# remydubois/illico

Measured on NVIDIA B200. Metric: gene_x_group_tests_per_s, higher is better.
Workload: dtype f32 keys / int64 ranks / f64 epilogue

## Files before the change

### illico_b200/csrc/fused.cu

```cuda
#include "common.cuh"
#include "epilogue.cuh"
#include "tma.cuh"

#include <stdlib.h>

namespace illico {

int launch_stage_dense_list(const float* X, long long ld, int gene_lb, const int* list, const int* n_list_dev, const int* mode_dev,
                            int want_mode, const illico_plan_t* plan, float* ir_vals, uint32_t* ir_cnt, cudaStream_t stream);
int launch_stage_dense_tma_if(const float* X, long long ld, int gene_lb, int b, const illico_plan_t* plan, float* ir_vals,
                              uint32_t* ir_cnt, int seg_lo, int seg_hi, cudaStream_t stream, int segs_per_cta_req,
                              const int* mode_dev, int want_mode);
int launch_stage_csr_if(const float*, const int32_t*, const long long*, int, int, const illico_plan_t*, float*, uint32_t*, void*, size_t,
                        const int*, int, cudaStream_t);
int launch_stage_csr_list(const float*, const int32_t*, const long long*, int, int, const int*, const int*, int, int,
                          const illico_plan_t*, float*, uint32_t*, cudaStream_t);
int launch_ovo_mapped(const float*, const uint32_t*, int, const int*, const int*, int, const illico_plan_t*, const illico_flags_t*, double*,
                      long long, void*, size_t, const illico_debug_t*, cudaStream_t);
int launch_ovr_mapped(const float*, const uint32_t*, int, const int*, const int*, int, const illico_plan_t*, const illico_flags_t*, double*,
                      long long, void*, size_t, const illico_debug_t*, cudaStream_t);
bool stage_dense_tma_ok(const float* X, long long ld, int gene_lb, int b, const illico_plan_t* plan);
int launch_stage_dense_tma(const float* X, long long ld, int gene_lb, int b, const illico_plan_t* plan, float* ir_vals,
                           uint32_t* ir_cnt, int seg_lo, int seg_hi, cudaStream_t stream, int segs_per_cta = 0);

namespace {

constexpr int FUSED_WARPS = 8;
constexpr int FUSED_LANES = FUSED_WARPS * 32;
constexpr int FUSED_THREADS = FUSED_LANES + 32;
constexpr int DCAP = 12;
constexpr long long PAIR_MAX = 208063;

struct Gtab {
    float* key;
    uint32_t* mult;
    uint32_t* wgt;
    double* fval;
    uint32_t* nnz;
    unsigned long long* tie;
    double* sum;
    int* n_bad;
    int* list;
    int* cmap;
    unsigned char* bad;
    unsigned char* cls;
    unsigned char* mode;
    uint32_t* wm;
    double* gc;
    int Gs;
};
constexpr int DW = 64;
constexpr int CLS_NARROW = 1, CLS_IDENT = 2, CLS_WANTS_WIDE = 4;
constexpr int WIDE_FROM = 11;
constexpr int HB_NONE = 0, HB_LIST = 1, HB_ALL = 2;
constexpr int GC_MU = 0, GC_NRNT = 1, GC_PROD12 = 2, GC_DENOM = 3, GC_INV_NT = 4, GC_N = 5;

size_t gtab_bytes(int b, int G) {
    const size_t bs = (size_t)((b + 63) & ~63), Gs = (size_t)((G + 63) & ~63);
    return bs * ((size_t)DCAP * 20 + 4 + 8 + 8 + 1 + 8 + 2 + (size_t)DW * 2) + Gs * 8 * GC_N + 1024;
}
Gtab gtab_carve(void* ws, int b, int G) {
    const size_t bs = (size_t)((b + 63) & ~63), Gs = (size_t)((G + 63) & ~63);
    char* p = reinterpret_cast<char*>((reinterpret_cast<uintptr_t>(ws) + 255) & ~(uintptr_t)255);
    Gtab c;
    c.Gs = (int)Gs;
    c.gc = reinterpret_cast<double*>(p); p += Gs * 8 * GC_N;
    c.fval = reinterpret_cast<double*>(p); p += bs * 8 * DCAP;
    c.tie = reinterpret_cast<unsigned long long*>(p); p += bs * 8;
    c.sum = reinterpret_cast<double*>(p); p += bs * 8;
    c.key = reinterpret_cast<float*>(p); p += bs * 4 * DCAP;
    c.mult = reinterpret_cast<uint32_t*>(p); p += bs * 4 * DCAP;
    c.wgt = reinterpret_cast<uint32_t*>(p); p += bs * 4 * DCAP;
    c.nnz = reinterpret_cast<uint32_t*>(p); p += bs * 4;
    c.n_bad = reinterpret_cast<int*>(p); p += 64;
    c.list = reinterpret_cast<int*>(p); p += bs * 4;
    c.cmap = reinterpret_cast<int*>(p); p += bs * 4;
    c.wm = reinterpret_cast<uint32_t*>(p); p += bs * 2 * DW;
    c.bad = reinterpret_cast<unsigned char*>(p); p += bs;
    c.cls = reinterpret_cast<unsigned char*>(p); p += bs;
    c.mode = reinterpret_cast<unsigned char*>(p);
    return c;
}

constexpr float ROUND_MAGIC = 12582912.0f;
constexpr uint32_t ROUND_MAGIC_BITS = 0x4B400000u;
__device__ __forceinline__ uint32_t count_bin(float v, bool& ok) {
    const float tt = __fadd_rn(v, ROUND_MAGIC);
    const uint32_t q1 = __float_as_uint(tt) - (ROUND_MAGIC_BITS + 1u);
    ok = (__fsub_rn(tt, ROUND_MAGIC) == v) && (q1 < (uint32_t)DW);
    return q1;
}

__global__ void __launch_bounds__(256) fused_ctab_kernel(const float* __restrict__ ir_vals, const uint32_t* __restrict__ ir_cnt,
                                                         int b, const illico_plan_t pl, int seg_lo, int seg_hi, int is_log1p,
                                                         Gtab gt, int bs, int wide_on) {
    __shared__ uint32_t wh[8][DW];
    const int lane = threadIdx.x & 31, wl = threadIdx.x >> 5;
    const int warp = (blockIdx.x * blockDim.x + threadIdx.x) >> 5, nwarps = (gridDim.x * blockDim.x) >> 5;
    const int S = pl.n_segments;
    for (int j = warp; j < b; j += nwarps) {
        float mykey = 0.0f;
        uint32_t mycnt = 0;
        int D = 0;
        bool nbad = false;
        bool general = false;
        for (int s = seg_lo; s < seg_hi && !nbad; ++s) {
            const int c = (int)ir_cnt[(long long)j * S + s];
            const float* src = ir_vals + (long long)j * pl.slot_cap + pl.seg_base[s];
            for (int i0 = 0; i0 < c && !nbad; i0 += 32) {
                const bool valid = i0 + lane < c;
                const float v = valid ? src[i0 + lane] : 0.0f;
                if (__any_sync(FULL, valid && !(v > 0.0f))) { nbad = general = true; break; }
                const unsigned same = __match_any_sync(FULL, __float_as_uint(v));
                const bool leader = valid && (__ffs(same) - 1 == lane);
                const uint32_t n = (uint32_t)__popc(same);
                unsigned leaders = __ballot_sync(FULL, leader);
                while (leaders) {
                    const int l = __ffs(leaders) - 1;
                    leaders &= leaders - 1;
                    const float vv = __shfl_sync(FULL, v, l);
                    const uint32_t nn = __shfl_sync(FULL, n, l);
                    const unsigned hit = __ballot_sync(FULL, lane < D && mykey == vv);
                    if (hit) {
                        if (lane == __ffs(hit) - 1) mycnt += nn;
                    } else if (D < DCAP) {
                        if (lane == D) { mykey = vv; mycnt = nn; }
                        ++D;
                    } else {
                        nbad = true;
                        break;
                    }
                }
            }
        }
        bool ident = wide_on != 0 && !general;
        if (ident) {
            wh[wl][lane] = 0u;
            wh[wl][lane + 32] = 0u;
            __syncwarp();
            if (!nbad) {
                bool okv = true;
                const uint32_t q1 = count_bin(mykey, okv);
                if (__any_sync(FULL, lane < D && !okv)) ident = false;
                else if (lane < D) wh[wl][q1] = mycnt;
            } else {
                for (int s = seg_lo; s < seg_hi && ident; ++s) {
                    const int c = (int)ir_cnt[(long long)j * S + s];
                    const float* src = ir_vals + (long long)j * pl.slot_cap + pl.seg_base[s];
                    for (int i0 = 0; i0 < c; i0 += 32) {
                        const bool valid = i0 + lane < c;
                        const float v = valid ? src[i0 + lane] : 0.0f;
                        bool okv;
                        const uint32_t q1 = count_bin(v, okv);
                        if (__any_sync(FULL, valid && !okv)) { ident = false; break; }
                        const unsigned same = __match_any_sync(FULL, __float_as_uint(v));
                        if (valid && (__ffs(same) - 1 == lane)) wh[wl][q1] += (uint32_t)__popc(same);
                        __syncwarp();
                    }
                }
            }
            __syncwarp();
        }
        int cls = nbad ? 0 : CLS_NARROW;
        if (ident) {
            const uint32_t c0 = wh[wl][lane], c1 = wh[wl][lane + 32];
            if (__any_sync(FULL, (c0 | c1) > 0xffffu)) {
                ident = false;
            } else {
                const uint32_t e0 = wh[wl][2 * lane], e1 = wh[wl][2 * lane + 1];
                gt.wm[(long long)lane * bs + j] = e0 | (e1 << 16);
                cls |= CLS_IDENT;
                if (nbad || D >= WIDE_FROM) cls |= CLS_WANTS_WIDE;
            }
        }
        __syncwarp();
        if (lane == 0) gt.cls[j] = (unsigned char)cls;
        if (nbad) continue;
        int pos = 0;
        for (int t = 0; t < D; ++t) pos += (__shfl_sync(FULL, mykey, t) < mykey) ? 1 : 0;
        const bool mine = lane < D;
        if (mine) { gt.key[(long long)pos * bs + j] = mykey; gt.mult[(long long)pos * bs + j] = mycnt; }
        if (lane >= D && lane < DCAP) { gt.key[(long long)lane * bs + j] = 0.0f; gt.mult[(long long)lane * bs + j] = 0u; }
        const uint32_t nnz = warp_sum<uint32_t>(mine ? mycnt : 0u);
        const unsigned long long tie = warp_sum_u64(mine ? (unsigned long long)cube_minus((long long)mycnt) : 0ull);
        const double sum = warp_sum_f64(mine ? (double)mycnt * fc_value(mykey, is_log1p) : 0.0);
        if (lane == 0) { gt.nnz[j] = nnz; gt.tie[j] = tie; gt.sum[j] = sum; }
    }
}

__global__ void __launch_bounds__(256) fused_mode_kernel(int b, Gtab gt) {
    const int j = blockIdx.x * blockDim.x + threadIdx.x;
    const int c = (j < b) ? gt.cls[j] : 0;
    const bool tile_wide = __syncthreads_or((c & CLS_WANTS_WIDE) != 0) != 0;
    const int mode = (tile_wide && (c & CLS_IDENT)) ? 1 : 0;
    const bool bad = j < b && mode == 0 && !(c & CLS_NARROW);
    if (j < b) { gt.mode[j] = (unsigned char)mode; gt.bad[j] = bad ? 1 : 0; }
    const int nb = __syncthreads_count(bad);
    if (threadIdx.x == 0 && nb) atomicAdd(gt.n_bad, nb);
}

template <int ROWS, int STAGES, int BUF>
struct FusedLayout {
    static constexpr int ROW_BYTES = FUSED_LANES * 4;
    static constexpr int STAGE_BYTES = ROWS * ROW_BYTES;
    static constexpr int RING_OFF = 0;
    static constexpr int NZ_OFF = STAGES * STAGE_BYTES;
    static constexpr int KEY_OFF = NZ_OFF + BUF * ROW_BYTES;
    static constexpr int HIST_OFF = KEY_OFF + DCAP * ROW_BYTES;
    static constexpr int BAR_OFF = HIST_OFF + DCAP * FUSED_LANES * 2;
    static constexpr int BYTES = BAR_OFF + 2 * STAGES * 8;
};

template <int ROWS, int STAGES, int BUF, int MINB, bool OVO>
__global__ void __launch_bounds__(FUSED_THREADS, MINB) fused_pass_kernel(const float* __restrict__ X, long long ld, int gene_lb,
                                                                         int b, const illico_plan_t pl, int groups_per_cta,
                                                                         Gtab gt, int bs, unsigned long long* __restrict__ rec,
                                                                         long long gstride, int share_1024) {
    using L = FusedLayout<ROWS, STAGES, BUF>;
    static_assert(32 % ROWS == 0 && BUF > ROWS, "layout");
    extern __shared__ __align__(128) unsigned char smem[];
    const uint32_t smem_a = (uint32_t)__cvta_generic_to_shared(smem);
    const uint32_t bars = smem_a + L::BAR_OFF;
    const int t = threadIdx.x, lane = t & 31, w = t >> 5;
    const int G = pl.n_groups, ref = OVO ? pl.ref_group : -1;
    const int gy0 = blockIdx.y * groups_per_cta, gy1 = min(G, gy0 + groups_per_cta);
    const int p_begin = pl.seg_pos[pl.group_seg[gy0]], p_end = pl.seg_pos[pl.group_seg[gy1]];
// ... 223 lines not shown
        const int p_end = pl.seg_pos[pl.group_seg[gy1]];
        k.ref_in = ref >= k.gy0 && ref < gy1;
        k.ref_p0 = k.ref_in ? pl.seg_pos[pl.group_seg[ref]] : 0;
        k.ref_len = k.ref_in ? pl.seg_pos[pl.group_seg[ref + 1]] - k.ref_p0 : 0;
        k.nv = p_end - k.p_begin - k.ref_len;
        return k;
    };

    if (w == FUSED_WARPS) {
        uint64_t policy;
        asm volatile("createpolicy.fractional.L2::evict_first.b64 %0, 1.0;" : "=l"(policy));
        const char* base = reinterpret_cast<const char*>(X + gene_lb + g0);
        const unsigned long long ldb = (unsigned long long)ld * 4ull;
        int k = 0;
        for (int c = blockIdx.y; c < n_chunks; c += gridDim.y) {
            const Chunk ch = chunk_of(c);
            auto row_of = [&](int i) {
                int p = ch.p_begin + i;
                if (ch.ref_in && p >= ch.ref_p0) p += ch.ref_len;
                return pl.perm[p];
            };
            int myrow = (lane < ch.nv) ? row_of(lane) : 0;
            for (int i0 = 0; i0 < ch.nv; i0 += 32) {
                const int nxt = (i0 + 32 + lane < ch.nv) ? row_of(i0 + 32 + lane) : 0;
                const int nrows = min(32, ch.nv - i0);
#pragma unroll
                for (int q = 0; q < 32 / ROWS; ++q, ++k) {
                    if (q * ROWS >= nrows) break;
                    const int slot = k % STAGES;
                    const uint32_t full = bars + 8 * slot, empty = bars + 8 * (STAGES + slot);
                    mbar_wait_backoff(empty, ((k / STAGES) & 1) ^ 1);
                    const int rows_here = min(ROWS, nrows - q * ROWS);
                    if (lane == 0) mbar_expect_tx(full, (uint32_t)rows_here * row_bytes);
                    __syncwarp();
                    const int u = lane - q * ROWS;
                    if (u >= 0 && u < rows_here)
                        bulk_g2s(smem_a + L::RING_OFF + slot * L::STAGE_BYTES + u * L::ROW_BYTES,
                                 base + (unsigned long long)(uint32_t)myrow * ldb, row_bytes, full, policy);
                }
                myrow = nxt;
            }
        }
        return;
    }

    const int j = g0 + t;
    const bool in_batch = j < b;
    const bool mine = in_batch && gt.bad[j] == 0 && gt.mode[j] == 1;
    const uint32_t hist_a = smem_a + L::HIST_OFF + (uint32_t)(w >> 1) * 128u + (uint32_t)lane * 4u + (uint32_t)(w & 1) * 2u;
    const uint32_t atab_a = smem_a + L::ATAB_OFF + t * 4;
    constexpr uint32_t BIN_BYTES = FUSED_LANES * 2;
    auto lds_f = [](uint32_t a) { float v; asm volatile("ld.shared.f32 %0, [%1];" : "=f"(v) : "r"(a)); return v; };
    auto lds_u = [](uint32_t a) { uint32_t v; asm volatile("ld.shared.u32 %0, [%1];" : "=r"(v) : "r"(a) : "memory"); return v; };
    auto sts_u = [](uint32_t a, uint32_t v) { asm volatile("st.shared.u32 [%0], %1;" ::"r"(a), "r"(v) : "memory"); };
    auto lds_h = [](uint32_t a) { uint32_t v; asm volatile("ld.shared.u16 %0, [%1];" : "=r"(v) : "r"(a) : "memory"); return v; };
    auto sts_h = [](uint32_t a, uint32_t v) { asm volatile("st.shared.u16 [%0], %1;" ::"r"(a), "r"(v) : "memory"); };
    {
        const uint32_t* wm_j = gt.wm + (in_batch ? j : 0);
#pragma unroll 8
        for (int q = 0; q < DW / 2; ++q) {
            sts_h(hist_a + (2 * q) * BIN_BYTES, 0u);
            sts_h(hist_a + (2 * q + 1) * BIN_BYTES, 0u);
            sts_u(atab_a + q * L::ROW_BYTES, mine ? __ldg(wm_j + (long long)q * bs) : 0u);
        }
    }
    bool bad = false;

    auto take = [&](float v) {
        bool ok;
        const uint32_t q1 = count_bin(v, ok);
        const uint32_t a = hist_a + q1 * BIN_BYTES;
        asm volatile(
            "{ .reg .pred p; .reg .u32 h;\n"
            "setp.ne.u32 p, %1, 0;\n"
            "@p ld.shared.u16 h, [%0];\n"
            "@p add.u32 h, h, 1;\n"
            "@p st.shared.u16 [%0], h; }"
            ::"r"(a), "r"((uint32_t)ok) : "memory");
        bad |= !ok && v != 0.0f;
    };
    auto close_group = [&](int g) {
        uint32_t m = 0, s1 = 0, above = 0;
        unsigned long long u2 = 0, tie = 0;
        auto bin = [&](uint32_t ha, uint32_t a, int q) {
            const uint32_t bq = lds_h(ha);
            if (bq) {
                sts_h(ha, 0u);
                u2 += (unsigned long long)bq * (2u * above + a);
                tie += (unsigned long long)(a * bq) * (3u * (a + bq));
                tie += (unsigned long long)(bq * bq) * bq;
                s1 += bq * (uint32_t)(q + 1);
                m += bq;
            }
            above += a;
        };
#pragma unroll 4
        for (int q = DW / 2 - 1; q >= 0; --q) {
            const uint32_t ab = lds_u(atab_a + q * L::ROW_BYTES);
            bin(hist_a + (2 * q + 1) * BIN_BYTES, ab >> 16, 2 * q + 1);
            bin(hist_a + (2 * q) * BIN_BYTES, ab & 0xffffu, 2 * q);
        }
        if (mine && !bad) {
            unsigned long long* o = rec + (long long)g * gstride + (long long)j * 3;
            o[0] = u2 | ((unsigned long long)m << WIDE_M_SHIFT);
            o[1] = tie - m;
            o[2] = (unsigned long long)s1;
        }
    };

    const uint32_t ring_a = smem_a + L::RING_OFF + t * 4;
    int slot = 0;
    uint32_t parity = 0;
    for (int c = blockIdx.y; c < n_chunks; c += gridDim.y) {
        const Chunk ch = chunk_of(c);
        if (ch.nv <= 0) continue;
        auto group_end_v = [&](int gg) {
            return pl.seg_pos[pl.group_seg[gg + 1]] - ch.p_begin - ((ch.ref_in && gg > ref) ? ch.ref_len : 0);
        };
        int g = (ch.gy0 == ref) ? ch.gy0 + 1 : ch.gy0;
        int gend = group_end_v(g);
        for (int i = 0; i < ch.nv; i += ROWS) {
            mbar_wait(bars + 8 * slot, parity);
            const uint32_t src = ring_a + slot * L::STAGE_BYTES;
            if (i + ROWS <= gend) {
                float v[ROWS];
#pragma unroll
                for (int u = 0; u < ROWS; ++u) v[u] = lds_f(src + u * L::ROW_BYTES);
#pragma unroll
                for (int u = 0; u < ROWS; ++u) take(v[u]);
            } else {
                const int nr = min(ROWS, ch.nv - i);
#pragma unroll 1
                for (int u = 0; u < nr; ++u) {
                    if (i + u == gend) {
                        close_group(g);
                        ++g;
                        if (g == ref) ++g;
                        gend = group_end_v(g);
                    }
                    take(lds_f(src + u * L::ROW_BYTES));
                }
            }
            __syncwarp();
            if (lane == 0) mbar_arrive(bars + 8 * (STAGES + slot));
            if (++slot == STAGES) { slot = 0; parity ^= 1u; }
        }
        close_group(g);
    }
    if (mine && bad) gt.bad[j] = 1;
}

template <bool OVO>
__global__ void __launch_bounds__(128) fused_gene_kernel(int b, const illico_plan_t pl, illico_flags_t fl, Gtab gt, int bs,
                                                         double* dbg_tie, long long* dbg_tie_exact) {
    const int j = blockIdx.x * blockDim.x + threadIdx.x;
    if (j >= b || gt.bad[j]) return;
    if (OVO && gt.mode[j] == 1) {
        unsigned long long nnz = 0, tie = 0, sum = 0;
        for (int q = 0; q < DW; ++q) {
            const unsigned long long c = (gt.wm[(long long)(q >> 1) * bs + j] >> (16 * (q & 1))) & 0xffffu;
            nnz += c;
            tie += (unsigned long long)cube_minus((long long)c);
            sum += c * (unsigned long long)(q + 1);
        }
        gt.nnz[j] = (uint32_t)nnz;
        gt.tie[j] = tie;
        gt.sum[j] = (double)sum;
        return;
    }
    float key[DCAP];
    int order[DCAP];
    int D = 0;
    for (int q = 0; q < DCAP; ++q) {
        const float kq = gt.key[(long long)q * bs + j];
        if (kq == 0.0f) break;
        int a = D - 1;
        while (a >= 0 && key[order[a]] > kq) { order[a + 1] = order[a]; --a; }
        key[q] = kq;
        order[a + 1] = q;
        ++D;
    }
    for (int q = D; q < DCAP; ++q) { gt.wgt[(long long)q * bs + j] = 0u; gt.fval[(long long)q * bs + j] = 0.0; }
    if (OVO) {
        unsigned long long above = 0, nnz = 0, tie = 0;
        for (int a = D - 1; a >= 0; --a) {
            const int q = order[a];
            const unsigned long long c = gt.mult[(long long)q * bs + j];
            gt.wgt[(long long)q * bs + j] = (uint32_t)(2ull * above + c);
            gt.fval[(long long)q * bs + j] = fc_value(key[q], fl.is_log1p);
            above += c;
        }
        double sum = 0.0;
        for (int a = 0; a < D; ++a) {
            const int q = order[a];
            const unsigned long long c = gt.mult[(long long)q * bs + j];
            nnz += c;
            tie += (unsigned long long)cube_minus((long long)c);
            sum += (double)c * gt.fval[(long long)q * bs + j];
        }
        gt.nnz[j] = (uint32_t)nnz;
        gt.tie[j] = tie;
        gt.sum[j] = sum;
        return;
    }
    const long long n = pl.n_cells;
    const bool sparse_order = fl.tie_order == ILLICO_TIES_SPARSE;
    unsigned long long nnz = 0;
    for (int q = 0; q < D; ++q) nnz += gt.mult[(long long)q * bs + j];
    const long long n0 = n - (long long)nnz;
    unsigned long long lo = (unsigned long long)n0, t_exact = 0;
    double total = 0.0;
    const unsigned long long zterm = (unsigned long long)cube_minus(n0);
    double walk = sparse_order ? 0.0 : (double)(long long)zterm;
    for (int a = 0; a < D; ++a) {
        const int q = order[a];
        const unsigned long long c = gt.mult[(long long)q * bs + j];
        gt.wgt[(long long)q * bs + j] = (uint32_t)(2ull * lo + c + 1ull);
        const double f = fc_value(key[q], fl.is_log1p);
        gt.fval[(long long)q * bs + j] = f;
        total += (double)c * f;
        const unsigned long long t3 = (unsigned long long)cube_minus((long long)c);
        t_exact += t3;
        walk += (double)(long long)t3;
        lo += c;
    }
    double tie;
    if (sparse_order) {
        const double x = (double)n0;
        tie = __dadd_rn(((double)t_exact >= TWO53) ? walk : (double)t_exact, __dsub_rn(__dmul_rn(__dmul_rn(x, x), x), x));
    } else {
        tie = ((double)t_exact + (double)zterm >= TWO53) ? walk : (double)(t_exact + zterm);
    }
    gt.nnz[j] = (uint32_t)(n0 + 1);
    gt.sum[j] = total;
    const double tie_corr = __dsub_rn(1.0, __ddiv_rn(fl.tie_correct ? tie : 0.0, (double)(n * (n - 1) * (n + 1))));
    gt.tie[j] = (unsigned long long)__double_as_longlong(tie_corr);
    if (dbg_tie) dbg_tie[j] = tie;
    if (dbg_tie_exact) dbg_tie_exact[j] = (long long)(t_exact + zterm);
}

template <bool OVO>
__global__ void __launch_bounds__(256) fused_group_kernel(const illico_plan_t pl, Gtab gt) {
    const int g = blockIdx.x * blockDim.x + threadIdx.x;
    if (g >= pl.n_groups) return;
    const long long n = pl.n_cells, n_t = pl.group_size[g];
    const long long n_r = OVO ? (long long)pl.group_size[pl.ref_group] : n - n_t;
    const long long nn = n_r + n_t;
    gt.gc[GC_MU * gt.Gs + g] = (double)(n_r * n_t) / 2.0;
    gt.gc[GC_NRNT * gt.Gs + g] = (double)(n_r * n_t);
    gt.gc[GC_PROD12 * gt.Gs + g] = __ddiv_rn((double)(n_r * n_t * (n_r + n_t + 1)), 12.0);
    gt.gc[GC_DENOM * gt.Gs + g] = (double)(nn * (nn - 1) * (nn + 1));
    gt.gc[GC_INV_NT * gt.Gs + g] = 1.0 / (double)n_t;
}

constexpr int EPI_GROUPS = 16;
template <bool OVO, bool WIDE, bool SCORE>
__global__ void __launch_bounds__(256, 3) fused_epilogue_kernel(int b, const illico_plan_t pl, const illico_flags_t fl, Gtab gt,
                                                             int bs, double* __restrict__ results, long long gstride,
                                                             long long* dbg_u2, double* dbg_tie, long long* dbg_tie_exact,
                                                             int share_1024) {
    __shared__ double gcs[GC_N][EPI_GROUPS];
    __shared__ int nts[EPI_GROUPS];
    const int G = pl.n_groups, ref = pl.ref_group;
    const int ga = blockIdx.y * EPI_GROUPS, gb = min(G, ga + EPI_GROUPS);
    if (threadIdx.x < GC_N * EPI_GROUPS) {
        const int c = threadIdx.x / EPI_GROUPS, k = threadIdx.x % EPI_GROUPS;
        if (ga + k < gb) gcs[c][k] = gt.gc[c * gt.Gs + ga + k];
    } else if (threadIdx.x < GC_N * EPI_GROUPS + EPI_GROUPS) {
        const int k = threadIdx.x - GC_N * EPI_GROUPS;
        if (ga + k < gb) nts[k] = pl.group_size[ga + k];
    }
    __syncthreads();
    const int j = blockIdx.x * blockDim.x + threadIdx.x;
    if (j >= b || gt.bad[j]) return;
    if ((long long)gt.n_bad[0] * 1024 > (long long)b * share_1024) return;
    if ((gt.mode[j] == 1) != WIDE) return;
    uint32_t wgt[WIDE ? 1 : DCAP], mult[(OVO && !WIDE) ? DCAP : 1];
    double fval[WIDE ? 1 : DCAP];
    if (!WIDE) {
#pragma unroll
        for (int q = 0; q < DCAP; ++q) {
            wgt[WIDE ? 0 : q] = gt.wgt[(long long)q * bs + j];
            fval[WIDE ? 0 : q] = gt.fval[(long long)q * bs + j];
            if (OVO) mult[(OVO && !WIDE) ? q : 0] = gt.mult[(long long)q * bs + j];
        }
    }
    const long long n = pl.n_cells;
    const double cc = fl.use_continuity ? 0.5 : 0.0;
    const long long g_nnz = gt.nnz[j];
    const unsigned long long g_tie = gt.tie[j];
    const double g_sum = gt.sum[j];
    const long long n_ref = OVO ? (long long)pl.group_size[ref] : 0;
    const double ovr_tie_corr = __longlong_as_double((long long)g_tie);
    const double ovo_rsum = OVO ? (fl.group_sums ? fl.group_sums[(long long)ref * b + j] : g_sum) : 0.0;
    const double ovo_mean_r = OVO ? ovo_rsum / (double)n_ref : 0.0;
    const double ovo_inv_mean_r = 1.0 / ovo_mean_r;
    for (int g = ga; g < gb; ++g) {
        const int k = g - ga;
        const long long n_t = nts[k];
        const long long n_r = OVO ? n_ref : n - n_t;
        double* o = results + (long long)g * gstride + (long long)j * 3;
        const long long di = (long long)g * b + j;
        if (OVO && g == ref) {
            o[0] = 1.0; o[1] = -1.0; o[2] = (ovo_mean_r == 0.0) ? INFINITY : ovo_mean_r / ovo_mean_r;
            if (SCORE) fl.scores[(long long)g * fl.score_group_stride + j] = 0.0;
            if (dbg_u2) dbg_u2[di] = -2;
            if (dbg_tie) dbg_tie[di] = 0.0;
            if (dbg_tie_exact) dbg_tie_exact[di] = 0;
            continue;
        }
        const unsigned long long* r = reinterpret_cast<const unsigned long long*>(o);
        const unsigned long long wds[3] = {r[0], r[1], r[2]};
        unsigned long long acc = 0, tie_nz = 0;
        uint32_t m = 0;
        double sum = 0.0;
        if (WIDE) {
            acc = wds[0] & ((1ull << WIDE_M_SHIFT) - 1ull);
            m = (uint32_t)(wds[0] >> WIDE_M_SHIFT);
            tie_nz = wds[1];
            sum = (double)wds[2];
        } else {
#pragma unroll
            for (int q = 0; q < DCAP; ++q) {
                const uint32_t bq = (uint32_t)(wds[q >> 2] >> (16 * (q & 3))) & 0xffffu;
                if (bq) {
                    acc += (unsigned long long)bq * wgt[WIDE ? 0 : q];
                    sum += (double)bq * fval[WIDE ? 0 : q];
                    m += bq;
                    if (OVO) {
                        const unsigned long long a = mult[(OVO && !WIDE) ? q : 0];
                        tie_nz += bq * (3ull * a * a - 1ull + bq * (3ull * a + bq));
                    }
                }
            }
        }
        const long long z_t = n_t - (long long)m;
        double p, U, fc;
        if (OVO) {
            const long long zeros_r = n_r - g_nnz;
            if (fl.group_sums) sum = fl.group_sums[(long long)g * b + j];
            const long long Z = zeros_r + z_t;
            const unsigned long long u2 = acc + (unsigned long long)(z_t * (2ll * g_nnz + zeros_r));
            const unsigned long long tie_exact = g_tie + tie_nz + (unsigned long long)cube_minus(Z);
            const double tie = (double)tie_exact;
            U = (double)u2 * 0.5;
            const double tie_corr = __dsub_rn(1.0, __ddiv_rn(fl.tie_correct ? tie : 0.0, gcs[GC_DENOM][k]));
            p = pval_core(gcs[GC_NRNT][k], gcs[GC_MU][k], gcs[GC_PROD12][k], tie_corr, U, cc, fl.alternative);
            if (SCORE) fl.scores[(long long)g * fl.score_group_stride + j] = score_core(gcs[GC_MU][k], gcs[GC_PROD12][k], tie_corr, U);
            fc = (ovo_mean_r == 0.0) ? INFINITY : (sum * gcs[GC_INV_NT][k]) * ovo_inv_mean_r;
            if (dbg_u2) dbg_u2[di] = (long long)u2;
            if (dbg_tie) dbg_tie[di] = tie;
            if (dbg_tie_exact) dbg_tie_exact[di] = (long long)tie_exact;
        } else {
            const unsigned long long R2 = acc + (unsigned long long)z_t * (unsigned long long)g_nnz;
            const long long u2 = 2 * n_r * n_t + n_t * (n_t + 1) - (long long)R2;
            U = (double)u2 * 0.5;
            p = pval_core(gcs[GC_NRNT][k], gcs[GC_MU][k], gcs[GC_PROD12][k], ovr_tie_corr, U, cc, fl.alternative);
            if (SCORE)
                fl.scores[(long long)g * fl.score_group_stride + j] = score_core(gcs[GC_MU][k], gcs[GC_PROD12][k], ovr_tie_corr, U);
            const bool all_here = (long long)m == n - (g_nnz - 1);
            const double mu_t = sum * gcs[GC_INV_NT][k], mu_r = all_here ? 0.0 : (g_sum - sum) / (double)(n - n_t);
            fc = (mu_r == 0.0) ? INFINITY : mu_t / mu_r;
            if (dbg_u2) dbg_u2[di] = u2;
        }
        o[0] = p; o[1] = U; o[2] = fc;
    }
}

constexpr int CSRF_THREADS = 1024;
constexpr int CSRF_TILE = 8192;

__device__ __forceinline__ int gtab_slot(float* gkey, int bs, float v) {
    int q = (int)v - 1;
    if (q >= 0 && q < DCAP && __ldcg(gkey + (long long)q * bs) == v) return q;
    if (!(v > 0.0f)) return -1;
    for (q = 0; q < DCAP; ++q) {
        float k = __ldcg(gkey + (long long)q * bs);
        if (k == 0.0f) {
            const unsigned old = atomicCAS(reinterpret_cast<unsigned*>(gkey + (long long)q * bs), 0u, __float_as_uint(v));
            k = old ? __uint_as_float(old) : v;
        }
        if (k == v) return q;
    }
    return -1;
}

__global__ void fused_seed_kernel(Gtab gt, int bs, int identity) {
    const int i = blockIdx.x * blockDim.x + threadIdx.x;
    if (i >= bs) return;
#pragma unroll
    for (int q = 0; q < DCAP; ++q) {
        gt.key[(long long)q * bs + i] = identity ? (float)(q + 1) : 0.0f;
        gt.mult[(long long)q * bs + i] = 0u;
    }
    gt.bad[i] = 0;
    gt.mode[i] = 0;
    if (i == 0) *gt.n_bad = 0;
}

__global__ void fused_zero_multi_kernel(int b, const illico_plan_t pl, unsigned long long* __restrict__ rec, long long gstride) {
    const int g = blockIdx.y;
    if (pl.group_seg[g + 1] - pl.group_seg[g] < 2) return;
    for (int i = blockIdx.x * blockDim.x + threadIdx.x; i < 3 * b; i += gridDim.x * blockDim.x) rec[(long long)g * gstride + i] = 0ull;
}

template <bool OVO>
__global__ void __launch_bounds__(CSRF_THREADS, 1) fused_csr_pass_kernel(const float* __restrict__ data, const int32_t* __restrict__ indices,
                                                                        const long long* __restrict__ indptr, int gene_lb, int b,
                                                                        const illico_plan_t pl, Gtab gt, int bs,
                                                                        unsigned long long* __restrict__ rec, long long gstride) {
    extern __shared__ __align__(16) uint32_t hist[];
    const int t = threadIdx.x, lane = t & 31, w = t >> 5;
    const int s = blockIdx.y, g = pl.seg_group[s];
    const int j_lo = blockIdx.x * CSRF_TILE, ng = min(CSRF_TILE, b - j_lo);
    __shared__ int stop;
    if (t == 0) stop = 8 * *reinterpret_cast<volatile int*>(gt.n_bad) > b;
    for (int i = t; i < ng * 6; i += CSRF_THREADS) hist[i] = 0u;
    __syncthreads();
    if (stop) return;
    const int c_lo = gene_lb + j_lo, c_hi = c_lo + ng;
    const int p0 = pl.seg_pos[s], p1 = pl.seg_pos[s + 1];
    constexpr int NW = CSRF_THREADS / 32;
    long long my_e0 = 0, my_e1 = 0;
    {
        const int p = p0 + w + lane * NW;
        if (p < p1) {
            const long long r = pl.perm[p];
            my_e0 = indptr[r];
            my_e1 = indptr[r + 1];
        }
    }
    for (int p = p0 + w, k = 0; p < p1; p += NW, ++k) {
        if (8 * *reinterpret_cast<volatile int*>(gt.n_bad) > b) break;
        if (k == 32) {
            const int pp = p + lane * NW;
            my_e0 = my_e1 = 0;
            if (pp < p1) { const long long r = pl.perm[pp]; my_e0 = indptr[r]; my_e1 = indptr[r + 1]; }
            k = 0;
        }
        long long e0 = __shfl_sync(FULL, my_e0, k);
        const long long e1 = __shfl_sync(FULL, my_e1, k);
        if (c_lo > 0) {
            long long lo = e0, hi = e1;
            while (lo < hi) { const long long mid = (lo + hi) >> 1; if (indices[mid] < c_lo) lo = mid + 1; else hi = mid; }
            e0 = lo;
        }
        for (long long e = e0 + lane; ; e += 128) {
            int c[4];
            float v[4], kq[4];
#pragma unroll
            for (int u = 0; u < 4; ++u) c[u] = (e + 32 * u < e1) ? __ldcs(indices + e + 32 * u) : 0x7fffffff;
#pragma unroll
            for (int u = 0; u < 4; ++u) v[u] = (e + 32 * u < e1) ? __ldcs(data + e + 32 * u) : 0.0f;
            if (__all_sync(FULL, c[0] >= c_hi)) break;
#pragma unroll
            for (int u = 0; u < 4; ++u) if (c[u] >= c_hi) v[u] = 0.0f;
#pragma unroll
            for (int u = 0; u < 4; ++u) {
                const int q = min(max((int)v[u] - 1, 0), DCAP - 1);
                kq[u] = (v[u] != 0.0f) ? __ldcg(gt.key + (long long)q * bs + j_lo + (c[u] - c_lo)) : 0.0f;
            }
#pragma unroll
            for (int u = 0; u < 4; ++u) {
                if (v[u] != 0.0f) {
                    const int jj = c[u] - c_lo;
                    int q = min(max((int)v[u] - 1, 0), DCAP - 1);
                    if (kq[u] != v[u]) q = gt.bad[j_lo + jj] ? -1 : gtab_slot(gt.key + j_lo + jj, bs, v[u]);
                    if (q >= 0) {
                        atomicAdd(&hist[jj * 6 + (q >> 1)], 1u << (16 * (q & 1)));
                    } else {
                        const int j = j_lo + jj;
                        const unsigned bit = 1u << (8 * (j & 3));
                        const unsigned old = atomicOr(reinterpret_cast<unsigned*>(gt.bad + (j & ~3)), bit);
                        if (!(old & bit)) atomicAdd(gt.n_bad, 1);
                    }
                }
            }
        }
    }
    __syncthreads();
    const bool multi = pl.group_seg[g + 1] - pl.group_seg[g] > 1;
    for (int jj = t; jj < ng; jj += CSRF_THREADS) {
        const int j = j_lo + jj;
        uint32_t wd[6];
#pragma unroll
        for (int k = 0; k < 6; ++k) wd[k] = hist[jj * 6 + k];
        if (OVO && g == pl.ref_group) {
#pragma unroll
            for (int q = 0; q < DCAP; ++q) {
                const uint32_t cq = (wd[q >> 1] >> (16 * (q & 1))) & 0xffffu;
                if (cq) atomicAdd(gt.mult + (long long)q * bs + j, cq);
            }
        } else if (!multi) {
            unsigned long long* o = rec + (long long)g * gstride + (long long)j * 3;
#pragma unroll
            for (int k = 0; k < 3; ++k) o[k] = (unsigned long long)wd[2 * k] | ((unsigned long long)wd[2 * k + 1] << 32);
        } else {
            uint32_t* o = reinterpret_cast<uint32_t*>(rec + (long long)g * gstride + (long long)j * 3);
#pragma unroll
            for (int k = 0; k < 6; ++k) if (wd[k]) atomicAdd(o + k, wd[k]);
        }
    }
}

__global__ void __launch_bounds__(256) fused_hist_sum_kernel(int b, int G, int groups_per_block, Gtab gt, int bs,
                                                             const unsigned long long* __restrict__ rec, long long gstride) {
    const int j = blockIdx.x * blockDim.x + threadIdx.x;
    if (j >= b || gt.bad[j]) return;
    const int ga = blockIdx.y * groups_per_block, gb = min(G, ga + groups_per_block);
    uint32_t acc[DCAP];
#pragma unroll
    for (int q = 0; q < DCAP; ++q) acc[q] = 0u;
    for (int g = ga; g < gb; ++g) {
        const unsigned long long* r = rec + (long long)g * gstride + (long long)j * 3;
        const unsigned long long wds[3] = {r[0], r[1], r[2]};
#pragma unroll
        for (int q = 0; q < DCAP; ++q) acc[q] += (uint32_t)((wds[q >> 2] >> (16 * (q & 3))) & 0xffffull);
    }
#pragma unroll
    for (int q = 0; q < DCAP; ++q)
        if (acc[q]) atomicAdd(gt.mult + (long long)q * bs + j, acc[q]);
}

__global__ void __launch_bounds__(1024) fused_list_kernel(int b, Gtab gt, int num, int den, int force_all) {
    __shared__ int wsum[32];
    __shared__ int base_s;
    const int t = threadIdx.x, lane = t & 31, w = t >> 5;
    if (t == 0) base_s = 0;
    __syncthreads();
    for (int j0 = 0; j0 < b; j0 += 1024) {
        const int j = j0 + t;
        const bool flag = j < b && gt.bad[j] != 0;
        const unsigned bal = __ballot_sync(FULL, flag);
        if (lane == 0) wsum[w] = __popc(bal);
        __syncthreads();
        int before = 0, total = 0;
        for (int ww = 0; ww < 32; ++ww) { const int c = wsum[ww]; if (ww < w) before += c; total += c; }
        const int base = base_s;
        if (j < b) {
            const int k = base + before + __popc(bal & ((1u << lane) - 1u));
            if (flag) gt.list[k] = j;
            gt.cmap[j] = flag ? k : -1;
        }
        __syncthreads();
        if (t == 0) base_s = base + total;
        __syncthreads();
    }
    const int n = base_s;
    const bool all = force_all || (long long)n * den > (long long)b * num;
    if (all && n > 0) {
        for (int j = t; j < b; j += 1024) { gt.list[j] = j; gt.cmap[j] = j; }
    }
    if (t == 0) {
        gt.n_bad[1] = (n == 0) ? 0 : (all ? b : n);
        gt.n_bad[2] = (n == 0) ? HB_NONE : (all ? HB_ALL : HB_LIST);
    }
}

int env_int(const char* name, int dflt) {
    const char* v = getenv(name);
    return v ? atoi(v) : dflt;
}
int list_share_1024() {
    const char* v = getenv("ILLICO_FUSED_LIST_SHARE");
    const double f = v ? atof(v) : 0.125;
    return (int)(f * 1024.0 + 0.5);
}

thread_local float g_last_fused_ms = -1.0f;

constexpr int PASS_ROWS = 1536;
constexpr int OVR_SAMPLE_CELLS = 16384;

template <bool OVO>
int run_fused(const float* X, long long ld, int gene_lb, int b, const illico_plan_t* plan, const illico_flags_t* flags,
              const illico_batch_buffers_t* buf, double* results, long long gstride, const illico_debug_t* dbg,
              cudaStream_t stream) {
    g_last_fused_ms = -1.0f;
    if (env_int(OVO ? "ILLICO_OVO_FUSED" : "ILLICO_OVR_FUSED", 1) == 0 || b <= 0) return -1;
    if (!stage_dense_tma_ok(X, ld, gene_lb, b, plan)) return -1;
    if (plan->max_target_group_size >= 65536 || plan->n_groups < 2 || plan->n_groups > 65535) return -1;
    if (OVO && (long long)plan->ref_group_size + plan->max_target_group_size > PAIR_MAX) return -1;
    if (!OVO && flags->group_sums) return -1;
    if (dbg) return -1;
    if (buf->workspace_bytes < gtab_bytes(b, plan->n_groups)) return -1;
    const int bs = (b + 63) & ~63;
    Gtab gt = gtab_carve(buf->workspace, b, plan->n_groups);

    const bool wide_on = OVO && !flags->is_log1p && env_int("ILLICO_FUSED_WIDE", 1) != 0;
    int seg_lo = plan->ref_seg_begin, seg_hi = plan->ref_seg_end;
    if (!OVO) {
        long long avg = plan->n_cells / plan->n_segments;
        if (avg < 1) avg = 1;
        seg_lo = 0;
        seg_hi = (int)((OVR_SAMPLE_CELLS + avg - 1) / avg);
        if (seg_hi < 1) seg_hi = 1;
        if (seg_hi > plan->n_segments) seg_hi = plan->n_segments;
    }
    ILLICO_CUDA_OK(cudaMemsetAsync(gt.n_bad, 0, 16 * sizeof(int), stream));
    {
        const int rc = launch_stage_dense_tma(X, ld, gene_lb, b, plan, buf->ir_vals, buf->ir_cnt, seg_lo, seg_hi, stream, 1);
        if (rc != 0) return rc;
        int blocks = (b + 7) / 8;
        if (blocks > 148 * 8) blocks = 148 * 8;
        ILLICO_LAUNCH("fused_ctab_kernel", stream, fused_ctab_kernel<<<blocks, 256, 0, stream>>>(buf->ir_vals, buf->ir_cnt, b, *plan, seg_lo, seg_hi, flags->is_log1p, gt, bs, wide_on ? 1 : 0));
        ILLICO_LAUNCH("fused_mode_kernel", stream, fused_mode_kernel<<<(b + FUSED_LANES - 1) / FUSED_LANES, FUSED_LANES, 0, stream>>>(b, gt));
        ILLICO_CUDA_OK(cudaGetLastError());
    }
    if (!OVO)
        ILLICO_CUDA_OK(cudaMemsetAsync(gt.mult, 0, (size_t)bs * DCAP * sizeof(uint32_t), stream));

    long long avg_g = plan->n_cells / plan->n_groups;
    if (avg_g < 1) avg_g = 1;
    int gpc = (int)(PASS_ROWS / avg_g);
    if (gpc < 1) gpc = 1;
    {
        using L = FusedLayout<8, 5, 16>;
        auto kern = fused_pass_kernel<8, 5, 16, 3, OVO>;
        ILLICO_CUDA_OK(cudaFuncSetAttribute(kern, cudaFuncAttributeMaxDynamicSharedMemorySize, (int)L::BYTES));
        const dim3 grid((unsigned)((b + FUSED_LANES - 1) / FUSED_LANES), (unsigned)((plan->n_groups + gpc - 1) / gpc));
        ILLICO_LAUNCH("fused_pass_kernel", stream, kern<<<grid, FUSED_THREADS, L::BYTES, stream>>>(X, ld, gene_lb, b, *plan, gpc, gt, bs,
                                                        reinterpret_cast<unsigned long long*>(results), gstride, list_share_1024()));
        ILLICO_CUDA_OK(cudaGetLastError());
    }
    if (wide_on) {
        auto kern = fused_wide_pass_kernel<8, 5, 2>;
        const int wide_smem = WideLayout<8, 5>::BYTES;
        ILLICO_CUDA_OK(cudaFuncSetAttribute(kern, cudaFuncAttributeMaxDynamicSharedMemorySize, wide_smem));
        const int tiles = (b + FUSED_LANES - 1) / FUSED_LANES, chunks = (plan->n_groups + gpc - 1) / gpc;
        int gy = (2 * 148) / tiles;
        if (gy < 1) gy = 1;
        if (gy > chunks) gy = chunks;
        const dim3 grid((unsigned)tiles, (unsigned)gy);
        ILLICO_LAUNCH("fused_wide_pass_kernel", stream, kern<<<grid, FUSED_THREADS, wide_smem, stream>>>(
                X, ld, gene_lb, b, *plan, gpc, gt, bs, reinterpret_cast<unsigned long long*>(results), gstride, list_share_1024()));
        ILLICO_CUDA_OK(cudaGetLastError());
    }
    g_last_fused_ms = 0.0f;

    ILLICO_LAUNCH("fused_group_kernel", stream, fused_group_kernel<OVO><<<(plan->n_groups + 255) / 256, 256, 0, stream>>>(*plan, gt));
    ILLICO_LAUNCH("fused_gene_kernel", stream, fused_gene_kernel<OVO><<<(b + 127) / 128, 128, 0, stream>>>(b, *plan, *flags, gt, bs, nullptr, nullptr));
    ILLICO_CUDA_OK(cudaGetLastError());
    const bool score = flags->scores != nullptr;
    auto epi = score ? fused_epilogue_kernel<OVO, false, true> : fused_epilogue_kernel<OVO, false, false>;
    ILLICO_LAUNCH("fused_epilogue_kernel", stream, epi<<<dim3((unsigned)((b + 255) / 256), (unsigned)((plan->n_groups + EPI_GROUPS - 1) / EPI_GROUPS)), 256, 0, stream>>>(
            b, *plan, *flags, gt, bs, results, gstride, nullptr, nullptr, nullptr, list_share_1024()));
    if (wide_on) {
        auto wepi = score ? fused_epilogue_kernel<OVO, true, true> : fused_epilogue_kernel<OVO, true, false>;
        ILLICO_LAUNCH("fused_wide_epilogue_kernel", stream, wepi<<<dim3((unsigned)((b + 255) / 256), (unsigned)((plan->n_groups + EPI_GROUPS - 1) / EPI_GROUPS)), 256, 0, stream>>>(
                b, *plan, *flags, gt, bs, results, gstride, nullptr, nullptr, nullptr, list_share_1024()));
    }
    ILLICO_CUDA_OK(cudaGetLastError());

    ILLICO_LAUNCH("fused_list_kernel", stream, fused_list_kernel<<<1, 1024, 0, stream>>>(b, gt, list_share_1024(), 1024, 0));
    ILLICO_CUDA_OK(cudaGetLastError());
    if (launch_stage_dense_list(X, ld, gene_lb, gt.list, gt.n_bad + 1, gt.n_bad + 2, HB_LIST, plan, buf->ir_vals, buf->ir_cnt, stream))
        return 1;
    if (launch_stage_dense_tma_if(X, ld, gene_lb, b, plan, buf->ir_vals, buf->ir_cnt, 0, plan->n_segments, stream, 0, gt.n_bad + 2,
                                  HB_ALL))
        return 1;
    const size_t tab = (gtab_bytes(b, plan->n_groups) + 255) & ~(size_t)255;
    if (buf->workspace_bytes <= tab) return 1;
    char* ws = reinterpret_cast<char*>(buf->workspace) + tab;
    const size_t ws_bytes = buf->workspace_bytes - tab;
    return OVO ? launch_ovo_mapped(buf->ir_vals, buf->ir_cnt, b, gt.n_bad + 1, gt.list, b, plan, flags, results, gstride, ws, ws_bytes,
                                   nullptr, stream)
               : launch_ovr_mapped(buf->ir_vals, buf->ir_cnt, b, gt.n_bad + 1, gt.list, b, plan, flags, results, gstride, ws, ws_bytes,
                                   nullptr, stream);
}

}

float ovo_fused_last_ms() { return g_last_fused_ms; }

size_t ovo_fused_workspace_bytes(int b, int n_groups) { return gtab_bytes(b, n_groups); }

int launch_ovo_dense_fused(const float* X, long long ld, int gene_lb, int b, const illico_plan_t* plan,
                           const illico_flags_t* flags, const illico_batch_buffers_t* buf, double* results, long long gstride,
                           const illico_debug_t* dbg, cudaStream_t stream) {
    return run_fused<true>(X, ld, gene_lb, b, plan, flags, buf, results, gstride, dbg, stream);
}

int launch_ovr_dense_fused(const float* X, long long ld, int gene_lb, int b, const illico_plan_t* plan,
                           const illico_flags_t* flags, const illico_batch_buffers_t* buf, double* results, long long gstride,
                           const illico_debug_t* dbg, cudaStream_t stream) {
    return run_fused<false>(X, ld, gene_lb, b, plan, flags, buf, results, gstride, dbg, stream);
}


namespace {

template <bool OVO>
int run_fused_csr(const float* data, const int32_t* indices, const long long* indptr, int gene_lb, int b,
                  const illico_plan_t* plan, const illico_flags_t* flags, const illico_batch_buffers_t* buf, double* results,
                  long long gstride, const illico_debug_t* dbg, cudaStream_t stream) {
    g_last_fused_ms = -1.0f;
    if (env_int(OVO ? "ILLICO_OVO_FUSED" : "ILLICO_OVR_FUSED", 1) == 0 || env_int("ILLICO_CSR_FUSED", 1) == 0 || b <= 0) return -1;
    if (plan->max_target_group_size >= 65536 || plan->n_groups < 2 || plan->n_groups > 65535 || plan->n_segments > 65535) return -1;
    if (OVO && (long long)plan->ref_group_size + plan->max_target_group_size > PAIR_MAX) return -1;
    if (!OVO && flags->group_sums) return -1;
    if (dbg) return -1;
    if (buf->workspace_bytes < gtab_bytes(b, plan->n_groups)) return -1;
    const int bs = (b + 63) & ~63;
    Gtab gt = gtab_carve(buf->workspace, b, plan->n_groups);
    unsigned long long* rec = reinterpret_cast<unsigned long long*>(results);
    const int G = plan->n_groups;

    ILLICO_CUDA_OK(cudaMemsetAsync(gt.n_bad, 0, 16 * sizeof(int), stream));
    ILLICO_LAUNCH("fused_seed_kernel", stream, fused_seed_kernel<<<(bs + 255) / 256, 256, 0, stream>>>(gt, bs, flags->is_log1p ? 0 : 1));
    ILLICO_LAUNCH("fused_zero_multi_kernel", stream, fused_zero_multi_kernel<<<dim3(8, (unsigned)G), 256, 0, stream>>>(b, *plan, rec, gstride));
    ILLICO_CUDA_OK(cudaGetLastError());
    {
        auto kern = fused_csr_pass_kernel<OVO>;
        const int tile = b < CSRF_TILE ? b : CSRF_TILE;
        const size_t smem = (size_t)tile * 24;
        ILLICO_CUDA_OK(cudaFuncSetAttribute(kern, cudaFuncAttributeMaxDynamicSharedMemorySize, (int)smem));
        const dim3 grid((unsigned)((b + CSRF_TILE - 1) / CSRF_TILE), (unsigned)plan->n_segments);
        ILLICO_LAUNCH("fused_csr_pass_kernel", stream, kern<<<grid, CSRF_THREADS, smem, stream>>>(data, indices, indptr, gene_lb, b, *plan, gt, bs, rec, gstride));
        ILLICO_CUDA_OK(cudaGetLastError());
    }
    g_last_fused_ms = 0.0f;
    if (!OVO) {
        const int gpb = 64;
        ILLICO_LAUNCH("fused_hist_sum_kernel", stream, fused_hist_sum_kernel<<<dim3((unsigned)((b + 255) / 256), (unsigned)((G + gpb - 1) / gpb)), 256, 0, stream>>>(b, G, gpb, gt, bs, rec,
                                                                                                                 gstride));
    }
    ILLICO_LAUNCH("fused_group_kernel", stream, fused_group_kernel<OVO><<<(plan->n_groups + 255) / 256, 256, 0, stream>>>(*plan, gt));
    ILLICO_LAUNCH("fused_gene_kernel", stream, fused_gene_kernel<OVO><<<(b + 127) / 128, 128, 0, stream>>>(b, *plan, *flags, gt, bs, nullptr, nullptr));
    auto epi = flags->scores ? fused_epilogue_kernel<OVO, false, true> : fused_epilogue_kernel<OVO, false, false>;
    ILLICO_LAUNCH("fused_epilogue_kernel", stream, epi<<<dim3((unsigned)((b + 255) / 256), (unsigned)((G + EPI_GROUPS - 1) / EPI_GROUPS)), 256, 0, stream>>>(
            b, *plan, *flags, gt, bs, results, gstride, nullptr, nullptr, nullptr, 128));
    ILLICO_CUDA_OK(cudaGetLastError());

    int share = list_share_1024();
    if (share > 128) share = 128;
    ILLICO_LAUNCH("fused_list_kernel", stream, fused_list_kernel<<<1, 1024, 0, stream>>>(b, gt, share, 1024, 0));
    ILLICO_CUDA_OK(cudaGetLastError());
    const size_t tab = (gtab_bytes(b, plan->n_groups) + 255) & ~(size_t)255;
    if (buf->workspace_bytes <= tab) return 1;
    char* ws = reinterpret_cast<char*>(buf->workspace) + tab;
    const size_t ws_bytes = buf->workspace_bytes - tab;
    const int max_list = (int)(((long long)b * share) / 1024) + 1;
    if (launch_stage_csr_list(data, indices, indptr, gene_lb, b, gt.cmap, gt.n_bad + 2, HB_LIST, max_list < b ? max_list : b, plan,
                              buf->ir_vals, buf->ir_cnt, stream)) return 1;
    if (launch_stage_csr_if(data, indices, indptr, gene_lb, b, plan, buf->ir_vals, buf->ir_cnt, ws, ws_bytes, gt.n_bad + 2, HB_ALL, stream))
        return 1;
    return OVO ? launch_ovo_mapped(buf->ir_vals, buf->ir_cnt, b, gt.n_bad + 1, gt.list, b, plan, flags, results, gstride, ws, ws_bytes,
                                   nullptr, stream)
               : launch_ovr_mapped(buf->ir_vals, buf->ir_cnt, b, gt.n_bad + 1, gt.list, b, plan, flags, results, gstride, ws, ws_bytes,
                                   nullptr, stream);
}

}

int launch_ovo_csr_fused(const float* data, const int32_t* indices, const long long* indptr, int gene_lb, int b,
                         const illico_plan_t* plan, const illico_flags_t* flags, const illico_batch_buffers_t* buf, double* results,
                         long long gstride, const illico_debug_t* dbg, cudaStream_t stream) {
    return run_fused_csr<true>(data, indices, indptr, gene_lb, b, plan, flags, buf, results, gstride, dbg, stream);
}
int launch_ovr_csr_fused(const float* data, const int32_t* indices, const long long* indptr, int gene_lb, int b,
                         const illico_plan_t* plan, const illico_flags_t* flags, const illico_batch_buffers_t* buf, double* results,
                         long long gstride, const illico_debug_t* dbg, cudaStream_t stream) {
    return run_fused_csr<false>(data, indices, indptr, gene_lb, b, plan, flags, buf, results, gstride, dbg, stream);
}

}
```

Before: 7.074 billion.

## Stage per-gene epilogue tables in shared memory and bound the loop by distinct-value count

Adds a per-gene count of used distinct values (nd), computed in the gene and CSR pass kernels. The epilogue uses a warp max of nd to cut the DCAP loop short. Per-gene weights, values and OVO tie constants move from registers to dynamic shared memory, and EPI_GROUPS doubles so each block covers more groups. This aims to lower register pressure and skip unused slots. In exchange it adds shared-memory traffic, lowers occupancy from the large smem footprint, and adds atomics for nd in the CSR pass.

```diff
diff --git a/illico_b200/csrc/fused.cu b/illico_b200/csrc/fused.cu
--- a/illico_b200/csrc/fused.cu
+++ b/illico_b200/csrc/fused.cu
@@ -37,6 +37,7 @@
     uint32_t* wgt;
     double* fval;
     uint32_t* nnz;
+    uint32_t* nd;
     unsigned long long* tie;
     double* sum;
     int* n_bad;
@@ -57,7 +58,7 @@
 
 size_t gtab_bytes(int b, int G) {
     const size_t bs = (size_t)((b + 63) & ~63), Gs = (size_t)((G + 63) & ~63);
-    return bs * ((size_t)DCAP * 20 + 4 + 8 + 8 + 1 + 8 + 2 + (size_t)DW * 2) + Gs * 8 * GC_N + 1024;
+    return bs * ((size_t)DCAP * 20 + 4 + 4 + 8 + 8 + 1 + 8 + 2 + (size_t)DW * 2) + Gs * 8 * GC_N + 1024;
 }
 Gtab gtab_carve(void* ws, int b, int G) {
     const size_t bs = (size_t)((b + 63) & ~63), Gs = (size_t)((G + 63) & ~63);
@@ -72,6 +73,7 @@
     c.mult = reinterpret_cast<uint32_t*>(p); p += bs * 4 * DCAP;
     c.wgt = reinterpret_cast<uint32_t*>(p); p += bs * 4 * DCAP;
     c.nnz = reinterpret_cast<uint32_t*>(p); p += bs * 4;
+    c.nd = reinterpret_cast<uint32_t*>(p); p += bs * 4;
     c.n_bad = reinterpret_cast<int*>(p); p += 64;
     c.list = reinterpret_cast<int*>(p); p += bs * 4;
     c.cmap = reinterpret_cast<int*>(p); p += bs * 4;
@@ -601,7 +603,7 @@
 
 template <bool OVO>
 __global__ void __launch_bounds__(128) fused_gene_kernel(int b, const illico_plan_t pl, illico_flags_t fl, Gtab gt, int bs,
-                                                         double* dbg_tie, long long* dbg_tie_exact) {
+                                                         int nd_seen, double* dbg_tie, long long* dbg_tie_exact) {
     const int j = blockIdx.x * blockDim.x + threadIdx.x;
     if (j >= b || gt.bad[j]) return;
     if (OVO && gt.mode[j] == 1) {
@@ -650,12 +652,19 @@
         gt.nnz[j] = (uint32_t)nnz;
         gt.tie[j] = tie;
         gt.sum[j] = sum;
+        gt.nd[j] = nd_seen ? min((uint32_t)D, gt.nd[j]) : (uint32_t)D;
         return;
     }
     const long long n = pl.n_cells;
     const bool sparse_order = fl.tie_order == ILLICO_TIES_SPARSE;
     unsigned long long nnz = 0;
-    for (int q = 0; q < D; ++q) nnz += gt.mult[(long long)q * bs + j];
+    int nd = 0;
+    for (int q = 0; q < D; ++q) {
+        const uint32_t c = gt.mult[(long long)q * bs + j];
+        nnz += c;
+        if (c) nd = q + 1;
+    }
+    gt.nd[j] = (uint32_t)nd;
     const long long n0 = n - (long long)nnz;
     unsigned long long lo = (unsigned long long)n0, t_exact = 0;
     double total = 0.0;
@@ -702,12 +711,15 @@
     gt.gc[GC_INV_NT * gt.Gs + g] = 1.0 / (double)n_t;
 }
 
-constexpr int EPI_GROUPS = 16;
+constexpr int EPI_GROUPS = 32;
+template <bool OVO>
+constexpr int epi_tab_bytes() { return (OVO ? 3 : 2) * DCAP * 256 * 8; }
 template <bool OVO, bool WIDE, bool SCORE>
 __global__ void __launch_bounds__(256, 3) fused_epilogue_kernel(int b, const illico_plan_t pl, const illico_flags_t fl, Gtab gt,
                                                              int bs, double* __restrict__ results, long long gstride,
                                                              long long* dbg_u2, double* dbg_tie, long long* dbg_tie_exact,
                                                              int share_1024) {
+    extern __shared__ unsigned long long tab[];
     __shared__ double gcs[GC_N][EPI_GROUPS];
     __shared__ int nts[EPI_GROUPS];
     const int G = pl.n_groups, ref = pl.ref_group;
@@ -720,18 +732,26 @@
         if (ga + k < gb) nts[k] = pl.group_size[ga + k];
     }
     __syncthreads();
+    if ((long long)gt.n_bad[0] * 1024 > (long long)b * share_1024) return;
     const int j = blockIdx.x * blockDim.x + threadIdx.x;
-    if (j >= b || gt.bad[j]) return;
-    if ((long long)gt.n_bad[0] * 1024 > (long long)b * share_1024) return;
-    if ((gt.mode[j] == 1) != WIDE) return;
-    uint32_t wgt[WIDE ? 1 : DCAP], mult[(OVO && !WIDE) ? DCAP : 1];
-    double fval[WIDE ? 1 : DCAP];
+    const bool live = j < b && gt.bad[j] == 0 && (gt.mode[j] == 1) == WIDE;
+    const int nd = (!WIDE && live) ? (int)gt.nd[j] : 0;
+    const int dw = WIDE ? 0 : __reduce_max_sync(FULL, nd);
+    if (!live) return;
+    unsigned long long* const tw = tab + threadIdx.x;
+    unsigned long long* const tc = tab + DCAP * 256 + threadIdx.x;
+    double* const tf = reinterpret_cast<double*>(tab + (OVO ? 2 : 1) * DCAP * 256) + threadIdx.x;
     if (!WIDE) {
-#pragma unroll
-        for (int q = 0; q < DCAP; ++q) {
-            wgt[WIDE ? 0 : q] = gt.wgt[(long long)q * bs + j];
-            fval[WIDE ? 0 : q] = gt.fval[(long long)q * bs + j];
-            if (OVO) mult[(OVO && !WIDE) ? q : 0] = gt.mult[(long long)q * bs + j];
+        for (int q = 0; q < nd; ++q) {
+            const uint32_t w = gt.wgt[(long long)q * bs + j];
+            if (OVO) {
+                const uint32_t a = gt.mult[(long long)q * bs + j];
+                tw[q * 256] = w | ((unsigned long long)(3u * a) << 32);
+                tc[q * 256] = 3ull * a * a - 1ull;
+            } else {
+                tw[q * 256] = w;
+            }
+            tf[q * 256] = gt.fval[(long long)q * bs + j];
         }
     }
     const long long n = pl.n_cells;
@@ -771,14 +791,16 @@
         } else {
 #pragma unroll
             for (int q = 0; q < DCAP; ++q) {
+                if (q == dw) break;
                 const uint32_t bq = (uint32_t)(wds[q >> 2] >> (16 * (q & 3))) & 0xffffu;
                 if (bq) {
-                    acc += (unsigned long long)bq * wgt[WIDE ? 0 : q];
-                    sum += (double)bq * fval[WIDE ? 0 : q];
+                    const unsigned long long wa = tw[q * 256];
+                    acc += (unsigned long long)bq * (uint32_t)wa;
+                    sum += (double)bq * tf[q * 256];
                     m += bq;
                     if (OVO) {
-                        const unsigned long long a = mult[(OVO && !WIDE) ? q : 0];
-                        tie_nz += bq * (3ull * a * a - 1ull + bq * (3ull * a + bq));
+                        const unsigned long long t = (unsigned long long)bq * ((uint32_t)(wa >> 32) + bq);
+                        tie_nz += (unsigned long long)bq * (tc[q * 256] + t);
                     }
                 }
             }
@@ -844,6 +866,7 @@
     }
     gt.bad[i] = 0;
     gt.mode[i] = 0;
+    gt.nd[i] = 0u;
     if (i == 0) *gt.n_bad = 0;
 }
 
@@ -940,14 +963,22 @@
                 const uint32_t cq = (wd[q >> 1] >> (16 * (q & 1))) & 0xffffu;
                 if (cq) atomicAdd(gt.mult + (long long)q * bs + j, cq);
             }
-        } else if (!multi) {
-            unsigned long long* o = rec + (long long)g * gstride + (long long)j * 3;
-#pragma unroll
-            for (int k = 0; k < 3; ++k) o[k] = (unsigned long long)wd[2 * k] | ((unsigned long long)wd[2 * k + 1] << 32);
         } else {
-            uint32_t* o = reinterpret_cast<uint32_t*>(rec + (long long)g * gstride + (long long)j * 3);
-#pragma unroll
-            for (int k = 0; k < 6; ++k) if (wd[k]) atomicAdd(o + k, wd[k]);
+            if (OVO) {
+                uint32_t hi = 0;
+#pragma unroll
+                for (int k = 0; k < 6; ++k) if (wd[k]) hi = 2 * k + ((wd[k] >> 16) ? 2 : 1);
+                if (hi > __ldcg(gt.nd + j)) atomicMax(gt.nd + j, hi);
+            }
+            if (!multi) {
+                unsigned long long* o = rec + (long long)g * gstride + (long long)j * 3;
+#pragma unroll
+                for (int k = 0; k < 3; ++k) o[k] = (unsigned long long)wd[2 * k] | ((unsigned long long)wd[2 * k + 1] << 32);
+            } else {
+                uint32_t* o = reinterpret_cast<uint32_t*>(rec + (long long)g * gstride + (long long)j * 3);
+#pragma unroll
+                for (int k = 0; k < 6; ++k) if (wd[k]) atomicAdd(o + k, wd[k]);
+            }
         }
     }
 }
@@ -1088,11 +1119,12 @@
     g_last_fused_ms = 0.0f;
 
     ILLICO_LAUNCH("fused_group_kernel", stream, fused_group_kernel<OVO><<<(plan->n_groups + 255) / 256, 256, 0, stream>>>(*plan, gt));
-    ILLICO_LAUNCH("fused_gene_kernel", stream, fused_gene_kernel<OVO><<<(b + 127) / 128, 128, 0, stream>>>(b, *plan, *flags, gt, bs, nullptr, nullptr));
+    ILLICO_LAUNCH("fused_gene_kernel", stream, fused_gene_kernel<OVO><<<(b + 127) / 128, 128, 0, stream>>>(b, *plan, *flags, gt, bs, 0, nullptr, nullptr));
     ILLICO_CUDA_OK(cudaGetLastError());
     const bool score = flags->scores != nullptr;
     auto epi = score ? fused_epilogue_kernel<OVO, false, true> : fused_epilogue_kernel<OVO, false, false>;
-    ILLICO_LAUNCH("fused_epilogue_kernel", stream, epi<<<dim3((unsigned)((b + 255) / 256), (unsigned)((plan->n_groups + EPI_GROUPS - 1) / EPI_GROUPS)), 256, 0, stream>>>(
+    ILLICO_CUDA_OK(cudaFuncSetAttribute(epi, cudaFuncAttributeMaxDynamicSharedMemorySize, epi_tab_bytes<OVO>()));
+    ILLICO_LAUNCH("fused_epilogue_kernel", stream, epi<<<dim3((unsigned)((b + 255) / 256), (unsigned)((plan->n_groups + EPI_GROUPS - 1) / EPI_GROUPS)), 256, epi_tab_bytes<OVO>(), stream>>>(
             b, *plan, *flags, gt, bs, results, gstride, nullptr, nullptr, nullptr, list_share_1024()));
     if (wide_on) {
         auto wepi = score ? fused_epilogue_kernel<OVO, true, true> : fused_epilogue_kernel<OVO, true, false>;
@@ -1175,9 +1207,10 @@
                                                                                                                  gstride));
     }
     ILLICO_LAUNCH("fused_group_kernel", stream, fused_group_kernel<OVO><<<(plan->n_groups + 255) / 256, 256, 0, stream>>>(*plan, gt));
-    ILLICO_LAUNCH("fused_gene_kernel", stream, fused_gene_kernel<OVO><<<(b + 127) / 128, 128, 0, stream>>>(b, *plan, *flags, gt, bs, nullptr, nullptr));
+    ILLICO_LAUNCH("fused_gene_kernel", stream, fused_gene_kernel<OVO><<<(b + 127) / 128, 128, 0, stream>>>(b, *plan, *flags, gt, bs, OVO ? 1 : 0, nullptr, nullptr));
     auto epi = flags->scores ? fused_epilogue_kernel<OVO, false, true> : fused_epilogue_kernel<OVO, false, false>;
-    ILLICO_LAUNCH("fused_epilogue_kernel", stream, epi<<<dim3((unsigned)((b + 255) / 256), (unsigned)((G + EPI_GROUPS - 1) / EPI_GROUPS)), 256, 0, stream>>>(
+    ILLICO_CUDA_OK(cudaFuncSetAttribute(epi, cudaFuncAttributeMaxDynamicSharedMemorySize, epi_tab_bytes<OVO>()));
+    ILLICO_LAUNCH("fused_epilogue_kernel", stream, epi<<<dim3((unsigned)((b + 255) / 256), (unsigned)((G + EPI_GROUPS - 1) / EPI_GROUPS)), 256, epi_tab_bytes<OVO>(), stream>>>(
             b, *plan, *flags, gt, bs, results, gstride, nullptr, nullptr, nullptr, 128));
     ILLICO_CUDA_OK(cudaGetLastError());
 
```

Measured after the change: 7.228 billion (median of 6 runs). 1.02x the previous value.
